# the3cloud/zktls

Measured on AMD Instinct MI355X. Metric: trace-cells/s, higher is better.
Workload: dtype u32

## Files before the change

### zktls_amd/csrc/hash.hip

```cpp
#include "poseidon2.cuh"
#include "poseidon2_coop.cuh"
#include "kernels.h"
#include "batch.h"
#include "p24chip.h"
#include "p24chip_rows.cuh"
#include "p2chip.h"

namespace zk {

hipError_t hash_upload_p2_tables(const P2Tables& t, hipStream_t s) { return p2_upload_tables(t, s); }

__device__ __forceinline__ uint32_t load_virtual(const LeafArgs& a, uint64_t row, uint32_t vc) {
    uint32_t off = vc;
#pragma unroll
    for (int m = 0; m < MAX_LEAF_MATS; m++) {
        if (m < a.nmats) {
            if (off < a.mats[m].width) return a.mats[m].ptr[row * a.mats[m].ld + off];
            off -= a.mats[m].width;
        }
    }
    return 0u;
}

__global__ void hash_rows16_kernel(LeafArgs a, uint32_t total_w);
struct hash_rows16_kernel_bargs { LeafArgs a; uint32_t total_w; static hash_rows16_kernel_bargs make(LeafArgs a, uint32_t total_w) { return hash_rows16_kernel_bargs{a, total_w}; } };
__global__ void hash_rows16_kernel_batch(const hash_rows16_kernel_bargs* __restrict__ zk_arr);
__global__ void compress_level16_kernel(const uint32_t* __restrict__ children, uint32_t* __restrict__ parents, uint32_t count);
struct compress_level16_kernel_bargs { const uint32_t* children; uint32_t* parents; uint32_t count; static compress_level16_kernel_bargs make(const uint32_t* children, uint32_t* parents, uint32_t count) { return compress_level16_kernel_bargs{children, parents, count}; } };
__global__ void compress_level16_kernel_batch(const compress_level16_kernel_bargs* __restrict__ zk_arr);
__global__ void compress_top16_kernel(uint32_t* tree, uint32_t count);
struct compress_top16_kernel_bargs { uint32_t* tree; uint32_t count; static compress_top16_kernel_bargs make(uint32_t* tree, uint32_t count) { return compress_top16_kernel_bargs{tree, count}; } };
__global__ void compress_top16_kernel_batch(const compress_top16_kernel_bargs* __restrict__ zk_arr);
__global__ void compress_sub16_kernel(uint32_t* tree, uint32_t count, uint32_t sub);
struct compress_sub16_kernel_bargs { uint32_t* tree; uint32_t count; uint32_t sub; static compress_sub16_kernel_bargs make(uint32_t* tree, uint32_t count, uint32_t sub) { return compress_sub16_kernel_bargs{tree, count, sub}; } };
__global__ void compress_sub16_kernel_batch(const compress_sub16_kernel_bargs* __restrict__ zk_arr);
__global__ void hash_sub16_kernel(LeafArgs a, uint32_t total_w, uint32_t sub);
struct hash_sub16_kernel_bargs { LeafArgs a; uint32_t total_w; uint32_t sub; static hash_sub16_kernel_bargs make(LeafArgs a, uint32_t total_w, uint32_t sub) { return hash_sub16_kernel_bargs{a, total_w, sub}; } };
__global__ void hash_sub16_kernel_batch(const hash_sub16_kernel_bargs* __restrict__ zk_arr);

__device__ __forceinline__ void hash_rows_generic_kernel_body(const LeafArgs& a, uint32_t total_w) {
    const uint64_t row = (uint64_t)blockIdx.x * blockDim.x + threadIdx.x;
    if (row >= a.height) return;
    uint32_t s[16];
#pragma unroll
    for (int i = 0; i < 16; i++) s[i] = 0u;
    for (uint32_t q = 0; q < total_w; q += 8) {
#pragma unroll
        for (int i = 0; i < 8; i++)
            if (q + i < total_w) s[i] = load_virtual(a, row, q + i);
        p2_permute_dev(s);
    }
    uint4* d = reinterpret_cast<uint4*>(a.digests + row * 8);
    d[0] = make_uint4(s[0], s[1], s[2], s[3]);
    d[1] = make_uint4(s[4], s[5], s[6], s[7]);
}
__global__ void __launch_bounds__(256) hash_rows_generic_kernel(LeafArgs a, uint32_t total_w) { hash_rows_generic_kernel_body(a, total_w); }
struct hash_rows_generic_kernel_bargs { LeafArgs a; uint32_t total_w; static hash_rows_generic_kernel_bargs make(LeafArgs a, uint32_t total_w) { return hash_rows_generic_kernel_bargs{a, total_w}; } };
__global__ void __launch_bounds__(256) hash_rows_generic_kernel_batch(const hash_rows_generic_kernel_bargs* __restrict__ zk_arr) { const hash_rows_generic_kernel_bargs& zk_b = zk_arr[blockIdx.z]; hash_rows_generic_kernel_body(zk_b.a, zk_b.total_w); }


template <bool MX>
__device__ __forceinline__ void hash_rows_vec_body(const uint32_t* __restrict__ mat, uint64_t ld, uint32_t width, uint64_t height, uint32_t* __restrict__ digests) {
    const uint64_t row = (uint64_t)blockIdx.x * blockDim.x + threadIdx.x;
    if (MX ? row - __lane_id() >= height : row >= height) return;
    const uint4* rp = reinterpret_cast<const uint4*>(mat + (row < height ? row : height - 1) * ld);
    uint32_t s[16];
#pragma unroll
    for (int i = 0; i < 16; i++) s[i] = 0u;
    for (uint32_t q = 0; q < width / 8; q++) {
        uint4 v0 = rp[2 * q], v1 = rp[2 * q + 1];
        s[0] = v0.x; s[1] = v0.y; s[2] = v0.z; s[3] = v0.w;
        s[4] = v1.x; s[5] = v1.y; s[6] = v1.z; s[7] = v1.w;
        if (MX) p2_permute_mx_dev(s); else p2_permute_dev(s);
    }
    if (width & 4u) {
        const uint4 v0 = rp[width / 4 - 1];
        s[0] = v0.x; s[1] = v0.y; s[2] = v0.z; s[3] = v0.w;
        if (MX) p2_permute_mx_dev(s); else p2_permute_dev(s);
    }
    if (row >= height) return;
    uint4* d = reinterpret_cast<uint4*>(digests + row * 8);
    d[0] = make_uint4(s[0], s[1], s[2], s[3]);
    d[1] = make_uint4(s[4], s[5], s[6], s[7]);
}
__device__ __forceinline__ void hash_rows_sponge_body(const uint32_t* __restrict__ mat, uint64_t ld, uint32_t width, uint64_t height, uint32_t* __restrict__ digests) {
    const uint64_t row = (uint64_t)blockIdx.x * blockDim.x + threadIdx.x;
    if (row - __lane_id() >= height) return;
    const uint4* rp = reinterpret_cast<const uint4*>(mat + (row < height ? row : height - 1) * ld);
    uint32_t s[16];
#pragma unroll
    for (int i = 0; i < 8; i++) { s[i] = 0u; s[8 + i] = (uint32_t)P2T.mx16.cap0[i]; }
    const uint32_t nb = width / 8, half = width & 4u;
    uint32_t q = 0;
    for (; q + 1 < nb; q++) {
        const uint4 v0 = rp[2 * q], v1 = rp[2 * q + 1];
        s[0] = v0.x; s[1] = v0.y; s[2] = v0.z; s[3] = v0.w;
        s[4] = v1.x; s[5] = v1.y; s[6] = v1.z; s[7] = v1.w;
        p2_permute_mx_form<P2MxForm::ABSORB>(s);
    }
    if (half && nb) {
        const uint4 v0 = rp[2 * q], v1 = rp[2 * q + 1];
        s[0] = v0.x; s[1] = v0.y; s[2] = v0.z; s[3] = v0.w;
        s[4] = v1.x; s[5] = v1.y; s[6] = v1.z; s[7] = v1.w;
        p2_permute_mx_form<P2MxForm::ABSORB_RATE>(s);
        q++;
    }
    if (width) {
        const uint4 v0 = rp[2 * q];
        s[0] = v0.x; s[1] = v0.y; s[2] = v0.z; s[3] = v0.w;
        if (!half) {
            const uint4 v1 = rp[2 * q + 1];
            s[4] = v1.x; s[5] = v1.y; s[6] = v1.z; s[7] = v1.w;
        }
        p2_permute_mx_form<P2MxForm::SQUEEZE>(s);
    }
    if (row >= height) return;
    uint4* d = reinterpret_cast<uint4*>(digests + row * 8);
    d[0] = make_uint4(s[0], s[1], s[2], s[3]);
    d[1] = make_uint4(s[4], s[5], s[6], s[7]);
}
__device__ __forceinline__ void hash_rows_vec_kernel_body(const uint32_t* __restrict__ mat, uint64_t ld, uint32_t width, uint64_t height, uint32_t* __restrict__ digests) { hash_rows_sponge_body(mat, ld, width, height, digests); }
__global__ void __launch_bounds__(256) __attribute__((amdgpu_waves_per_eu(5))) hash_rows_vec_kernel(const uint32_t* __restrict__ mat, uint64_t ld, uint32_t width, uint64_t height, uint32_t* __restrict__ digests) { hash_rows_vec_kernel_body(mat, ld, width, height, digests); }
struct hash_rows_vec_kernel_bargs { const uint32_t* mat; uint64_t ld; uint32_t width; uint64_t height; uint32_t* digests; static hash_rows_vec_kernel_bargs make(const uint32_t* mat, uint64_t ld, uint32_t width, uint64_t height, uint32_t* digests) { return hash_rows_vec_kernel_bargs{mat, ld, width, height, digests}; } };
__global__ void __launch_bounds__(256) __attribute__((amdgpu_waves_per_eu(5))) hash_rows_vec_kernel_batch(const hash_rows_vec_kernel_bargs* __restrict__ zk_arr) { const hash_rows_vec_kernel_bargs& zk_b = zk_arr[blockIdx.z]; hash_rows_vec_kernel_body(zk_b.mat, zk_b.ld, zk_b.width, zk_b.height, zk_b.digests); }
#ifdef ZKHIP_AB_HOOKS
__global__ void __launch_bounds__(256) hash_rows_vec_valu_kernel(const uint32_t* __restrict__ mat, uint64_t ld, uint32_t width, uint64_t height, uint32_t* __restrict__ digests) { hash_rows_vec_body<false>(mat, ld, width, height, digests); }
__global__ void __launch_bounds__(256) __attribute__((amdgpu_waves_per_eu(5))) hash_rows_vec_closed_kernel(const uint32_t* __restrict__ mat, uint64_t ld, uint32_t width, uint64_t height, uint32_t* __restrict__ digests) { hash_rows_vec_body<true>(mat, ld, width, height, digests); }
#endif

__device__ __forceinline__ void sponge_rows_vec(const LeafArgs& a, uint64_t row, uint32_t total_q, uint32_t s[16]) {
    int m = 0;
    uint32_t q = 0, nq = a.mats[0].width / 4;
    const uint4* rp = reinterpret_cast<const uint4*>(a.mats[0].ptr + row * a.mats[0].ld);
    for (uint32_t b = 0; b < total_q; b += 2) {
        while (q == nq) { m++; q = 0; nq = a.mats[m].width / 4; rp = reinterpret_cast<const uint4*>(a.mats[m].ptr + row * a.mats[m].ld); }
        const uint4 v0 = rp[q++];
        s[0] = v0.x; s[1] = v0.y; s[2] = v0.z; s[3] = v0.w;
        if (b + 1 < total_q) {
            while (q == nq) { m++; q = 0; nq = a.mats[m].width / 4; rp = reinterpret_cast<const uint4*>(a.mats[m].ptr + row * a.mats[m].ld); }
            const uint4 v1 = rp[q++];
            s[4] = v1.x; s[5] = v1.y; s[6] = v1.z; s[7] = v1.w;
        }
        p2_permute_dev(s);
    }
}
__device__ __forceinline__ void hash_rows_mvec_kernel_body(const LeafArgs& a, uint32_t total_q) {
    const uint64_t row = (uint64_t)blockIdx.x * blockDim.x + threadIdx.x;
    if (row >= a.height) return;
    uint32_t s[16];
#pragma unroll
    for (int i = 0; i < 16; i++) s[i] = 0u;
    sponge_rows_vec(a, row, total_q, s);
    uint4* d = reinterpret_cast<uint4*>(a.digests + row * 8);
    d[0] = make_uint4(s[0], s[1], s[2], s[3]);
    d[1] = make_uint4(s[4], s[5], s[6], s[7]);
}
__global__ void __launch_bounds__(256) hash_rows_mvec_kernel(LeafArgs a, uint32_t total_q) { hash_rows_mvec_kernel_body(a, total_q); }
struct hash_rows_mvec_kernel_bargs { LeafArgs a; uint32_t total_q; static hash_rows_mvec_kernel_bargs make(LeafArgs a, uint32_t total_q) { return hash_rows_mvec_kernel_bargs{a, total_q}; } };
__global__ void __launch_bounds__(256) hash_rows_mvec_kernel_batch(const hash_rows_mvec_kernel_bargs* __restrict__ zk_arr) { const hash_rows_mvec_kernel_bargs& zk_b = zk_arr[blockIdx.z]; hash_rows_mvec_kernel_body(zk_b.a, zk_b.total_q); }

__device__ __forceinline__ void compress_inject_mvec_kernel_body(const uint32_t* __restrict__ children, const LeafArgs& a, uint32_t total_q) {
    const uint64_t i = (uint64_t)blockIdx.x * blockDim.x + threadIdx.x;
    if (i >= a.height) return;
    const uint4* cp = reinterpret_cast<const uint4*>(children + 16 * i);
    const uint4 c0 = cp[0], c1 = cp[1], c2 = cp[2], c3 = cp[3];
    uint32_t s[16] = {c0.x, c0.y, c0.z, c0.w, c1.x, c1.y, c1.z, c1.w, c2.x, c2.y, c2.z, c2.w, c3.x, c3.y, c3.z, c3.w};
    uint32_t t[16];
#pragma unroll
    for (int k = 0; k < 16; k++) t[k] = 0u;
    p2_permute_dev(s);
    sponge_rows_vec(a, i, total_q, t);
#pragma unroll
    for (int k = 0; k < 8; k++) s[8 + k] = t[k];
    p2_permute_dev(s);
    uint4* d = reinterpret_cast<uint4*>(a.digests + i * 8);
    d[0] = make_uint4(s[0], s[1], s[2], s[3]);
    d[1] = make_uint4(s[4], s[5], s[6], s[7]);
}
__global__ void __launch_bounds__(256) compress_inject_mvec_kernel(const uint32_t* __restrict__ children, LeafArgs a, uint32_t total_q) { compress_inject_mvec_kernel_body(children, a, total_q); }
struct compress_inject_mvec_kernel_bargs { const uint32_t* children; LeafArgs a; uint32_t total_q; static compress_inject_mvec_kernel_bargs make(const uint32_t* children, LeafArgs a, uint32_t total_q) { return compress_inject_mvec_kernel_bargs{children, a, total_q}; } };
__global__ void __launch_bounds__(256) compress_inject_mvec_kernel_batch(const compress_inject_mvec_kernel_bargs* __restrict__ zk_arr) { const compress_inject_mvec_kernel_bargs& zk_b = zk_arr[blockIdx.z]; compress_inject_mvec_kernel_body(zk_b.children, zk_b.a, zk_b.total_q); }

static bool leaf_mats_vec(const LeafArgs& a) {
    for (int m = 0; m < a.nmats; m++) {
        const MatDesc& d = a.mats[m];
        if (d.width == 0 || d.width % 4 || d.ld % 4 || (reinterpret_cast<uintptr_t>(d.ptr) & 15)) return false;
    }
    return a.nmats >= 1;
}
hipError_t launch_compress_inject(const uint32_t* children, const LeafArgs& a, hipStream_t s) {
    if (a.height == 0) return hipSuccess;
    if (a.nmats < 1 || a.nmats > MAX_LEAF_MATS || !leaf_mats_vec(a)) return hipErrorInvalidValue;
    uint32_t total = 0;
    for (int m = 0; m < a.nmats; m++) total += a.mats[m].width;
    ZK_LAUNCH(compress_inject_mvec_kernel, compress_inject_mvec_kernel_batch, compress_inject_mvec_kernel_bargs, dim3((unsigned)((a.height + 255) / 256)), dim3(256), 0, s, children, a, total / 4);
    return hipGetLastError();
}
bool compress_inject_ok(const LeafArgs& a) { return a.height > coop_max_nodes() && leaf_mats_vec(a); }

hipError_t launch_hash_rows(const LeafArgs& a, hipStream_t s) {
    if (a.height == 0) return hipSuccess;
    if (a.nmats < 1 || a.nmats > MAX_LEAF_MATS) return hipErrorInvalidValue;
    uint32_t total = 0;
    for (int m = 0; m < a.nmats; m++) total += a.mats[m].width;
    if (a.height <= coop_max_nodes()) {
        const uint64_t threads = a.height * 16;
        ZK_LAUNCH(hash_rows16_kernel, hash_rows16_kernel_batch, hash_rows16_kernel_bargs, dim3((unsigned)((threads + 255) / 256)), dim3(256), 0, s, a, total);
        return hipGetLastError();
    }
    dim3 block(256), grid((unsigned)((a.height + 255) / 256));
    const MatDesc& m0 = a.mats[0];
    bool vec = a.nmats == 1 && m0.width % 4 == 0 && m0.ld % 4 == 0 &&
               (reinterpret_cast<uintptr_t>(m0.ptr) & 15) == 0;
#ifdef ZKHIP_AB_HOOKS
    static const bool valu = getenv("ZKHIP_HASH_VEC_VALU") != nullptr;
    if (vec && valu) {
        hash_rows_vec_valu_kernel<<<grid, block, 0, s>>>(m0.ptr, m0.ld, m0.width, a.height, a.digests);
        return hipGetLastError();
    }
    static const bool closed = getenv("ZKHIP_HASH_VEC_CLOSED") != nullptr;
    if (vec && closed) {
        hash_rows_vec_closed_kernel<<<grid, block, 0, s>>>(m0.ptr, m0.ld, m0.width, a.height, a.digests);
        return hipGetLastError();
    }
#endif
    if (vec)
        ZK_LAUNCH(hash_rows_vec_kernel, hash_rows_vec_kernel_batch, hash_rows_vec_kernel_bargs, grid, block, 0, s, m0.ptr, m0.ld, m0.width, a.height, a.digests);
    else if (leaf_mats_vec(a))
        ZK_LAUNCH(hash_rows_mvec_kernel, hash_rows_mvec_kernel_batch, hash_rows_mvec_kernel_bargs, grid, block, 0, s, a, total / 4);
    else
        ZK_LAUNCH(hash_rows_generic_kernel, hash_rows_generic_kernel_batch, hash_rows_generic_kernel_bargs, grid, block, 0, s, a, total);
    return hipGetLastError();
}

__device__ __forceinline__ void compress_node(const uint32_t* children, uint32_t* parent) {
    const uint4* cp = reinterpret_cast<const uint4*>(children);
    uint4 v0 = cp[0], v1 = cp[1], v2 = cp[2], v3 = cp[3];
    uint32_t s[16] = {v0.x, v0.y, v0.z, v0.w, v1.x, v1.y, v1.z, v1.w,
                      v2.x, v2.y, v2.z, v2.w, v3.x, v3.y, v3.z, v3.w};
    p2_permute_dev(s);
    uint4* d = reinterpret_cast<uint4*>(parent);
    d[0] = make_uint4(s[0], s[1], s[2], s[3]);
    d[1] = make_uint4(s[4], s[5], s[6], s[7]);
}

__device__ __forceinline__ void compress_level_kernel_body(const uint32_t* __restrict__ children, uint32_t* __restrict__ parents, uint64_t count) {
    const uint64_t i = (uint64_t)blockIdx.x * blockDim.x + threadIdx.x;
    if (i >= count) return;
    compress_node(children + 16 * i, parents + 8 * i);
}
__global__ void __launch_bounds__(256) compress_level_kernel(const uint32_t* __restrict__ children, uint32_t* __restrict__ parents, uint64_t count) { compress_level_kernel_body(children, parents, count); }
struct compress_level_kernel_bargs { const uint32_t* children; uint32_t* parents; uint64_t count; static compress_level_kernel_bargs make(const uint32_t* children, uint32_t* parents, uint64_t count) { return compress_level_kernel_bargs{children, parents, count}; } };
__global__ void __launch_bounds__(256) compress_level_kernel_batch(const compress_level_kernel_bargs* __restrict__ zk_arr) { const compress_level_kernel_bargs& zk_b = zk_arr[blockIdx.z]; compress_level_kernel_body(zk_b.children, zk_b.parents, zk_b.count); }

hipError_t launch_compress_level(const uint32_t* children, uint32_t* parents, uint64_t count, hipStream_t s) {
    if (count == 0) return hipSuccess;
    if (count <= coop_max_nodes()) {
        const uint64_t threads = count * 16;
        ZK_LAUNCH(compress_level16_kernel, compress_level16_kernel_batch, compress_level16_kernel_bargs, dim3((unsigned)((threads + 255) / 256)), dim3(256), 0, s, children, parents, (uint32_t)count);
        return hipGetLastError();
    }
    ZK_LAUNCH(compress_level_kernel, compress_level_kernel_batch, compress_level_kernel_bargs, dim3((unsigned)((count + 255) / 256)), dim3(256), 0, s, children, parents, count);
    return hipGetLastError();
}

__device__ __forceinline__ void inject_kernel_body(uint32_t* __restrict__ nodes, const uint32_t* __restrict__ extra, uint64_t count) {
    const uint64_t i = (uint64_t)blockIdx.x * blockDim.x + threadIdx.x;
    if (i >= count) return;
    const uint4* a = reinterpret_cast<const uint4*>(nodes + 8 * i);
    const uint4* b = reinterpret_cast<const uint4*>(extra + 8 * i);
    const uint4 v0 = a[0], v1 = a[1], v2 = b[0], v3 = b[1];
    uint32_t s[16] = {v0.x, v0.y, v0.z, v0.w, v1.x, v1.y, v1.z, v1.w, v2.x, v2.y, v2.z, v2.w, v3.x, v3.y, v3.z, v3.w};
    p2_permute_dev(s);
    uint4* d = reinterpret_cast<uint4*>(nodes + 8 * i);
    d[0] = make_uint4(s[0], s[1], s[2], s[3]);
    d[1] = make_uint4(s[4], s[5], s[6], s[7]);
}
__global__ void __launch_bounds__(256) inject_kernel(uint32_t* __restrict__ nodes, const uint32_t* __restrict__ extra, uint64_t count) { inject_kernel_body(nodes, extra, count); }
struct inject_kernel_bargs { uint32_t* nodes; const uint32_t* extra; uint64_t count; static inject_kernel_bargs make(uint32_t* nodes, const uint32_t* extra, uint64_t count) { return inject_kernel_bargs{nodes, extra, count}; } };
__global__ void __launch_bounds__(256) inject_kernel_batch(const inject_kernel_bargs* __restrict__ zk_arr) { const inject_kernel_bargs& zk_b = zk_arr[blockIdx.z]; inject_kernel_body(zk_b.nodes, zk_b.extra, zk_b.count); }

hipError_t launch_inject(uint32_t* nodes, const uint32_t* extra, uint64_t count, hipStream_t s) {
    if (count == 0) return hipSuccess;
    ZK_LAUNCH(inject_kernel, inject_kernel_batch, inject_kernel_bargs, dim3((unsigned)((count + 255) / 256)), dim3(256), 0, s, nodes, extra, count);
    return hipGetLastError();
}

__device__ __forceinline__ void compress_top_kernel_body(uint32_t* tree, uint32_t count) {
    uint32_t* level = tree;
    for (uint32_t n = count; n > 1; n >>= 1) {
        uint32_t* next = level + 8 * (size_t)n;
        for (uint32_t i = threadIdx.x; i < n / 2; i += blockDim.x) compress_node(level + 16 * (size_t)i, next + 8 * (size_t)i);
        __threadfence_block();
        __syncthreads();
        level = next;
    }
}
__global__ void __launch_bounds__(1024) compress_top_kernel(uint32_t* tree, uint32_t count) { compress_top_kernel_body(tree, count); }
struct compress_top_kernel_bargs { uint32_t* tree; uint32_t count; static compress_top_kernel_bargs make(uint32_t* tree, uint32_t count) { return compress_top_kernel_bargs{tree, count}; } };
__global__ void __launch_bounds__(1024) compress_top_kernel_batch(const compress_top_kernel_bargs* __restrict__ zk_arr) { const compress_top_kernel_bargs& zk_b = zk_arr[blockIdx.z]; compress_top_kernel_body(zk_b.tree, zk_b.count); }

hipError_t launch_compress_top(uint32_t* tree, uint32_t count, hipStream_t s) {
    if (count <= 1) return hipSuccess;
    if (count > COOP_TOP_NODES) return hipErrorInvalidValue;
    unsigned threads = count * 8 < 64 ? 64 : (count * 8 > 1024 ? 1024 : count * 8);
    ZK_LAUNCH(compress_top16_kernel, compress_top16_kernel_batch, compress_top16_kernel_bargs, dim3(1), dim3(threads), 0, s, tree, count);
    return hipGetLastError();
}

hipError_t launch_hash_sub(const LeafArgs& a, uint32_t sub, hipStream_t s) {
    if (sub < 2 || (sub & (sub - 1)) || a.height % sub || a.height > COOP_MAX_NODES || a.nmats < 1 || a.nmats > MAX_LEAF_MATS) return hipErrorInvalidValue;
    uint32_t total = 0;
    for (int m = 0; m < a.nmats; m++) total += a.mats[m].width;
    unsigned threads = sub * 8 < 64 ? 64 : (sub * 8 > 1024 ? 1024 : sub * 8);
    ZK_LAUNCH(hash_sub16_kernel, hash_sub16_kernel_batch, hash_sub16_kernel_bargs, dim3((unsigned)(a.height / sub)), dim3(threads), 0, s, a, total, sub);
    return hipGetLastError();
}
hipError_t launch_compress_sub(uint32_t* tree, uint32_t count, uint32_t sub, hipStream_t s) {
    if (sub < 2 || (sub & (sub - 1)) || count % sub || count > COOP_MAX_NODES) return hipErrorInvalidValue;
    unsigned threads = sub * 8 < 64 ? 64 : (sub * 8 > 1024 ? 1024 : sub * 8);
    ZK_LAUNCH(compress_sub16_kernel, compress_sub16_kernel_batch, compress_sub16_kernel_bargs, dim3(count / sub), dim3(threads), 0, s, tree, count, sub);
    return hipGetLastError();
}

__device__ __forceinline__ void compress_level16_kernel_body(const uint32_t* __restrict__ children, uint32_t* __restrict__ parents, uint32_t count) {
    const uint32_t gid = blockIdx.x * blockDim.x + threadIdx.x;
    const uint32_t node = gid >> 4;
    const int lane16 = threadIdx.x & 15;
    if (node >= count) return;
    const CoopConsts k = coop_load_consts(lane16);
    const uint32_t x = coop_permute(children[16 * (size_t)node + lane16], lane16, k);
    if (lane16 < 8) parents[8 * (size_t)node + lane16] = x;
}
__global__ void __launch_bounds__(256) compress_level16_kernel(const uint32_t* __restrict__ children, uint32_t* __restrict__ parents, uint32_t count) { compress_level16_kernel_body(children, parents, count); }
__global__ void __launch_bounds__(256) compress_level16_kernel_batch(const compress_level16_kernel_bargs* __restrict__ zk_arr) { const compress_level16_kernel_bargs& zk_b = zk_arr[blockIdx.z]; compress_level16_kernel_body(zk_b.children, zk_b.parents, zk_b.count); }

__device__ __forceinline__ void compress_top16_kernel_body(uint32_t* tree, uint32_t count) {
    const int lane16 = threadIdx.x & 15;
    const uint32_t grp = threadIdx.x >> 4, ngrp = blockDim.x >> 4;
    const CoopConsts k = coop_load_consts(lane16);
    uint32_t* level = tree;
    for (uint32_t n = count; n > 1; n >>= 1) {
        uint32_t* next = level + 8 * (size_t)n;
        for (uint32_t i = grp; i < n / 2; i += ngrp) {
            const uint32_t x = coop_permute(level[16 * (size_t)i + lane16], lane16, k);
            if (lane16 < 8) next[8 * (size_t)i + lane16] = x;
        }
        __threadfence_block();
        __syncthreads();
        level = next;
    }
}
__global__ void __launch_bounds__(1024) compress_top16_kernel(uint32_t* tree, uint32_t count) { compress_top16_kernel_body(tree, count); }
__global__ void __launch_bounds__(1024) compress_top16_kernel_batch(const compress_top16_kernel_bargs* __restrict__ zk_arr) { const compress_top16_kernel_bargs& zk_b = zk_arr[blockIdx.z]; compress_top16_kernel_body(zk_b.tree, zk_b.count); }

__device__ __forceinline__ void compress_sub16_kernel_body(uint32_t* tree, uint32_t count, uint32_t sub) {
    const int lane16 = threadIdx.x & 15;
    const uint32_t grp = threadIdx.x >> 4, ngrp = blockDim.x >> 4;
    const CoopConsts k = coop_load_consts(lane16);
    uint32_t* level = tree;
    uint32_t n = count, mine = sub;
    while (mine > 1) {
        uint32_t* next = level + 8 * (size_t)n;
        const size_t in0 = (size_t)blockIdx.x * mine, out0 = (size_t)blockIdx.x * (mine / 2);
        for (uint32_t i = grp; i < mine / 2; i += ngrp) {
            const uint32_t x = coop_permute(level[16 * (in0 / 2 + i) + lane16], lane16, k);
            if (lane16 < 8) next[8 * (out0 + i) + lane16] = x;
        }
        __threadfence_block();
        __syncthreads();
        level = next; n >>= 1; mine >>= 1;
    }
}
__global__ void __launch_bounds__(1024) compress_sub16_kernel(uint32_t* tree, uint32_t count, uint32_t sub) { compress_sub16_kernel_body(tree, count, sub); }
__global__ void __launch_bounds__(1024) compress_sub16_kernel_batch(const compress_sub16_kernel_bargs* __restrict__ zk_arr) { const compress_sub16_kernel_bargs& zk_b = zk_arr[blockIdx.z]; compress_sub16_kernel_body(zk_b.tree, zk_b.count, zk_b.sub); }
// ... 887 lines not shown
```

### zktls_amd/csrc/poseidon2.cuh

```cuda
#pragma once
#include "babybear.cuh"
#include "p2_params.h"

namespace zk {

struct P2Consts {
    uint32_t ext_rc[8][16];
    uint32_t int_rc[13];
    uint32_t diag[16];
    uint32_t ext_rcm[8][16];
    uint32_t int_rcm[13];
};
struct P2Raw {
    uint32_t ext16[8][16], int16[13], diag16[16];
    uint32_t ext24[8][24], int24[21], diag24[24];
};
constexpr P2Consts make_p2_consts(const P2Raw& raw) {
    P2Consts k{};
    for (int r = 0; r < 8; r++)
        for (int i = 0; i < 16; i++) k.ext_rc[r][i] = to_monty(raw.ext16[r][i]);
    for (int r = 0; r < 13; r++) k.int_rc[r] = to_monty(raw.int16[r]);
    for (int i = 0; i < 16; i++) k.diag[i] = to_monty(raw.diag16[i]);
    for (int r = 0; r < 8; r++)
        for (int i = 0; i < 16; i++) k.ext_rcm[r][i] = k.ext_rc[r][i] - P;
// ... 442 lines not shown
}
ZK_D void p2_m4_hl_dev(uint32_t& x0, uint32_t& x1, uint32_t& x2, uint32_t& x3) {
    const uint32_t t0 = dadd(x0, x1);
    const uint32_t t1 = dadd(x2, x3);
    const uint32_t t2 = dadd(ddbl(x1), t1);
    const uint32_t t3 = dadd(ddbl(x3), t0);
    const uint32_t t4 = dadd(ddbl(ddbl(t1)), t3);
    const uint32_t t5 = dadd(ddbl(ddbl(t0)), t2);
    x0 = dadd(t3, t5);
    x1 = t5;
    x2 = dadd(t2, t4);
    x3 = t4;
}
ZK_D void p2_external_linear_dev(uint32_t s[16]) {
    p2_m4_dev(s[0], s[1], s[2], s[3]);
    p2_m4_dev(s[4], s[5], s[6], s[7]);
    p2_m4_dev(s[8], s[9], s[10], s[11]);
    p2_m4_dev(s[12], s[13], s[14], s[15]);
    const uint32_t t0 = dadd(dadd(s[0], s[4]), dadd(s[8], s[12]));
    const uint32_t t1 = dadd(dadd(s[1], s[5]), dadd(s[9], s[13]));
    const uint32_t t2 = dadd(dadd(s[2], s[6]), dadd(s[10], s[14]));
    const uint32_t t3 = dadd(dadd(s[3], s[7]), dadd(s[11], s[15]));
#pragma unroll
    for (int b = 0; b < 16; b += 4) {
        s[b] = dadd(s[b], t0);
        s[b + 1] = dadd(s[b + 1], t1);
        s[b + 2] = dadd(s[b + 2], t2);
        s[b + 3] = dadd(s[b + 3], t3);
    }
}
#ifndef P2_INT_UNROLL
#define P2_INT_UNROLL 1
#endif
ZK_D int32_t p2_sbox_signed(int32_t t) {
    const int32_t x2 = dsmont(t, t);
    const int32_t x4 = dsmont(x2, x2);
    const int32_t x6 = dsmont(x4, x2);
    return dsmont(x6, t);
}
ZK_D void p2_internal_round_dev(int32_t v[16], int r, int32_t sh) {
    v[0] = p2_sbox_signed(v[0]);
    int64_t T = 0;
#pragma unroll
    for (int j = 0; j < 16; j++) T = dsmac_uniform(v[j], sh, T);
    const int32_t sum = dsmred(T);
    int64_t T2 = dsmac_s(sum, P2IK.k_sum, 0);
    v[0] = dsmred(dsmac_s(v[0], P2IK.diag[0], T2 + (int64_t)P2IK.rc_fold[r]));
#pragma unroll
    for (int i = 1; i < 16; i++) v[i] = dsmred(dsmac_s(v[i], P2IK.diag[i], T2));
}
ZK_D void p2_internal_pair_dev(int32_t v[16], int r, int32_t sh24) {
    int64_t A = 0;
#pragma unroll
    for (int i = 1; i < 16; i++) A = dsmac_uniform(v[i], P2PK.rs_mul[i], A);
    const int32_t u = p2_sbox_signed(v[0]);
    int64_t T = 0;
    T = dsmac_uniform(u, sh24, T);
#pragma unroll
    for (int j = 1; j < 16; j++) T = dsmac_uniform(v[j], sh24, T);
    const int32_t sum_t = dsmred(T);
    const int32_t v0 = dsmred(dsmac_s(u, P2IK.diag[0], dsmac_s(sum_t, P2PK.k_sum_a, 0) + (int64_t)P2IK.rc_fold[r]));
    A = dsmac_s(sum_t, P2PK.c15, A);
    const int32_t u2 = p2_sbox_signed(v0);
    A = dsmac_uniform(u2, P2PK.rs_mul[0], A);
    const int64_t T2 = dsmac_s(dsmred(A), P2PK.k_sum_b, 0);
    v[0] = dsmred(dsmac_s(u2, P2IK.diag[0], T2 + (int64_t)P2IK.rc_fold[r + 1]));
#pragma unroll
    for (int i = 1; i < 16; i++) v[i] = dsmred(dsmac_s(v[i], P2PK.d2[i], dsmac_s(sum_t, P2PK.e[i], T2)));
}
ZK_D void p2_internal_rounds_dev(uint32_t s[16]) {
    int32_t v[16];
#pragma unroll
    for (int i = 0; i < 16; i++) v[i] = (int32_t)s[i];
    int32_t sh, sh24;
    asm volatile("s_mov_b32 %0, 0x8000000" : "=s"(sh));
    asm volatile("s_mov_b32 %0, 0x1000000" : "=s"(sh24));
    p2_internal_round_dev(v, 0, sh);
    if (P2PK.pair) {
#pragma unroll P2_INT_UNROLL
        for (int r = 1; r < 13; r += 2) p2_internal_pair_dev(v, r, sh24);
    } else {
#pragma unroll P2_INT_UNROLL
        for (int r = 1; r < 13; r++) p2_internal_round_dev(v, r, sh);
    }
#pragma unroll
    for (int i = 0; i < 16; i++) s[i] = dcanon(v[i]);
}
ZK_D uint32_t p2_sbox_fold_dev(int32_t t, int64_t fold_biased) {
    const int32_t x2 = dsmont(t, t);
    const int32_t x4 = dsmont(x2, x2);
    const int32_t x6 = dsmont(x4, x2);
    return dred(dmred_lazy((uint64_t)dsmac(x6, t, fold_biased)));
}
ZK_D void p2_external_linear_signed_dev(uint32_t s[16]) {
    p2_m4_dev(s[0], s[1], s[2], s[3]);
    p2_m4_dev(s[4], s[5], s[6], s[7]);
    p2_m4_dev(s[8], s[9], s[10], s[11]);
    p2_m4_dev(s[12], s[13], s[14], s[15]);
    const uint32_t t0 = dadd(dadd(s[0], s[4]), dadd(s[8], s[12])) - P;
    const uint32_t t1 = dadd(dadd(s[1], s[5]), dadd(s[9], s[13])) - P;
    const uint32_t t2 = dadd(dadd(s[2], s[6]), dadd(s[10], s[14])) - P;
    const uint32_t t3 = dadd(dadd(s[3], s[7]), dadd(s[11], s[15])) - P;
#pragma unroll
    for (int b = 0; b < 16; b += 4) {
        s[b] += t0;
        s[b + 1] += t1;
        s[b + 2] += t2;
        s[b + 3] += t3;
    }
}
ZK_D void p2_permute_dev(uint32_t s[16]) {
    p2_external_linear_dev(s);
#pragma unroll
    for (int i = 0; i < 16; i++) s[i] += P2K.ext_rcm[0][i];
#pragma unroll 1
    for (int r = 0; r < 4; r++) {
#pragma unroll
        for (int i = 0; i < 16; i++) s[i] = p2_sbox_fold_dev((int32_t)s[i], P2EF.c[r][i]);
        p2_external_linear_signed_dev(s);
    }
    p2_internal_rounds_dev(s);
#pragma unroll
    for (int i = 0; i < 16; i++) s[i] += P2K.ext_rcm[4][i];
#pragma unroll 1
    for (int r = 4; r < 8; r++) {
#pragma unroll
        for (int i = 0; i < 16; i++) s[i] = p2_sbox_fold_dev((int32_t)s[i], P2EF.c[r][i]);
        p2_external_linear_signed_dev(s);
    }
#pragma unroll
    for (int i = 0; i < 16; i++) s[i] = dcanon((int32_t)s[i]);
}

typedef int p2mx_v4i __attribute__((ext_vector_type(4)));
typedef int p2mx_v16i __attribute__((ext_vector_type(16)));
constexpr int32_t MX_C24 = centered((uint32_t)(((uint64_t)1 << 56) % P));
constexpr uint32_t p2_me_entry(int i, int j) {
    return ((i >> 2) == (j >> 2) ? 2u : 1u) * (uint32_t)(0x1132u >> (4 * ((j - i) & 3)) & 15u);
}
constexpr uint32_t p2_mx_a_word(int lane, int idx) {
    const int m = lane & 31, h = lane >> 5, mb = idx >> 3, kb = (idx >> 2) & 1, r = idx & 3;
    return p2_me_entry(mx_elem((m >> 2) & 1, 4 * mb + (m >> 3)), mx_elem(h, 4 * kb + r)) << (8 * (m & 3));
}
struct P2MxA { uint32_t w[64][16]; };
constexpr P2MxA make_p2_mx_a() {
    P2MxA a{};
    for (int l = 0; l < 64; l++)
        for (int i = 0; i < 16; i++) a.w[l][i] = p2_mx_a_word(l, i);
    return a;
}
static_assert(p2_me_entry(0, 0) == 4 && p2_me_entry(0, 1) == 6 && p2_me_entry(1, 0) == 2 && p2_me_entry(3, 0) == 6 && p2_me_entry(4, 1) == 3,
              "M_E entries");
static __constant__ P2MxA d_p2_mx_a = make_p2_mx_a();
ZK_D void p2_mx_load_a(p2mx_v4i a[4]) {
    const uint4* p = reinterpret_cast<const uint4*>(d_p2_mx_a.w[__lane_id()]);
#pragma unroll
    for (int i = 0; i < 4; i++) { const uint4 v = p[i]; a[i] = p2mx_v4i{(int)v.x, (int)v.y, (int)v.z, (int)v.w}; }
}
ZK_D void p2_mx_layer_block(const uint32_t d[8], const p2mx_v4i a[4], int32_t w[8], int mb) {
    const p2mx_v4i b0 = {(int)d[0], (int)d[1], (int)d[2], (int)d[3]}, b1 = {(int)d[4], (int)d[5], (int)d[6], (int)d[7]};
    p2mx_v16i y = {};
    y = __builtin_amdgcn_mfma_i32_32x32x32_i8(a[2 * mb], b0, y, 0, 0, 0);
    y = __builtin_amdgcn_mfma_i32_32x32x32_i8(a[2 * mb + 1], b1, y, 0, 0, 0);
#pragma unroll
    for (int e = 0; e < 4; e++) {
        const uint32_t L = (uint32_t)y[4 * e] + ((uint32_t)y[4 * e + 1] << 8) + ((uint32_t)y[4 * e + 2] << 16);
        w[4 * mb + e] = dsmred((int64_t)((uint64_t)L << 32) + (int64_t)y[4 * e + 3] * MX_C24);
    }
}
ZK_D void p2_mx_layer(const uint32_t d[8], const p2mx_v4i a[4], int32_t w[8]) {
    p2_mx_layer_block(d, a, w, 0);
    p2_mx_layer_block(d, a, w, 1);
}
ZK_D uint32_t p2_sbox_mx_dev(int32_t t, int64_t fold_mx) {
    const int32_t x2 = dsmont(t, t);
    const int32_t x4 = dsmont(x2, x2);
    const int32_t x6 = dsmont(x4, x2);
    return dmred_lazy((uint64_t)dsmac(x6, t, fold_mx)) ^ 0x80808080u;
}
ZK_D void p2_mx_swap(uint32_t x[8], uint32_t y[8]) {
#pragma unroll
    for (int q = 0; q < 8; q++) {
        const auto r = __builtin_amdgcn_permlane32_swap(x[q], y[q], false, false);
        x[q] = r[0]; y[q] = r[1];
    }
}
ZK_D void p2_mx_full_rounds(int32_t wa[8], int32_t wb[8], int r0, int h) {
    p2mx_v4i a[4];
    p2_mx_load_a(a);
#pragma unroll 1
    for (int r = r0; r < r0 + 4; r++) {
        const int64_t* f = P2T.mx16.fold[r][h];
        uint32_t d[8];
#pragma unroll
        for (int q = 0; q < 8; q++) d[q] = p2_sbox_mx_dev(wa[q], f[q]);
        p2_mx_layer(d, a, wa);
#pragma unroll
        for (int q = 0; q < 8; q++) d[q] = p2_sbox_mx_dev(wb[q], f[q]);
        p2_mx_layer(d, a, wb);
    }
}
template <int BLOCKS>
ZK_D void p2_mx_last_rounds(int32_t wa[8], int32_t wb[8], int h, const int64_t* f7) {
    p2mx_v4i a[4];
    p2_mx_load_a(a);
    uint32_t d[8];
#pragma unroll 1
    for (int r = 4; r < 7; r++) {
        const int64_t* f = P2T.mx16.fold[r][h];
#pragma unroll
        for (int q = 0; q < 8; q++) d[q] = p2_sbox_mx_dev(wa[q], f[q]);
        p2_mx_layer(d, a, wa);
#pragma unroll
        for (int q = 0; q < 8; q++) d[q] = p2_sbox_mx_dev(wb[q], f[q]);
        p2_mx_layer(d, a, wb);
    }
#pragma unroll
    for (int q = 0; q < 8; q++) d[q] = p2_sbox_mx_dev(wa[q], f7[q]);
    if (BLOCKS & 1) p2_mx_layer_block(d, a, wa, 0);
    if (BLOCKS & 2) p2_mx_layer_block(d, a, wa, 1);
#pragma unroll
    for (int q = 0; q < 8; q++) d[q] = p2_sbox_mx_dev(wb[q], f7[q]);
    if (BLOCKS & 1) p2_mx_layer_block(d, a, wb, 0);
    if (BLOCKS & 2) p2_mx_layer_block(d, a, wb, 1);
}
enum class P2MxForm { CLOSED, ABSORB, ABSORB_RATE, SQUEEZE };
template <P2MxForm F>
ZK_D void p2_permute_mx_form(uint32_t s[16]) {
    constexpr bool SPONGE = F != P2MxForm::CLOSED;
    const int h = __lane_id() >> 5;
    uint32_t x[8], y[8];
    int32_t wa[8], wb[8];
#pragma unroll
    for (int q = 0; q < 8; q++) { x[q] = s[mx_elem(0, q)]; y[q] = s[mx_elem(1, q)]; }
    p2_mx_swap(x, y);
    {
        const uint32_t* c = P2T.mx16.in0[h];
        uint32_t da[8], db[8];
        p2mx_v4i a[4];
        p2_mx_load_a(a);
#pragma unroll
        for (int q = 0; q < 8; q++) {
            const uint32_t cq = SPONGE && q >= 4 ? 0x80808080u : c[q];
            da[q] = (x[q] + cq) ^ 0x80808080u; db[q] = (y[q] + cq) ^ 0x80808080u;
        }
        p2_mx_layer(da, a, wa);
        p2_mx_layer(db, a, wb);
    }
    p2_mx_full_rounds(wa, wb, 0, h);
#pragma unroll
    for (int q = 0; q < 8; q++) { x[q] = (uint32_t)wa[q]; y[q] = (uint32_t)wb[q]; }
    p2_mx_swap(x, y);
#pragma unroll
    for (int q = 0; q < 8; q++) { s[mx_elem(0, q)] = x[q]; s[mx_elem(1, q)] = y[q]; }
    p2_internal_rounds_dev(s);
#pragma unroll
    for (int q = 0; q < 8; q++) { x[q] = s[mx_elem(0, q)] + P2K.ext_rcm[4][mx_elem(0, q)]; y[q] = s[mx_elem(1, q)] + P2K.ext_rcm[4][mx_elem(1, q)]; }
    p2_mx_swap(x, y);
#pragma unroll
    for (int q = 0; q < 8; q++) { wa[q] = (int32_t)x[q]; wb[q] = (int32_t)y[q]; }
    if (!SPONGE) {
        p2_mx_full_rounds(wa, wb, 4, h);
#pragma unroll
        for (int q = 0; q < 8; q++) { x[q] = dcanon(wa[q]); y[q] = dcanon(wb[q]); }
        p2_mx_swap(x, y);
#pragma unroll
        for (int q = 0; q < 8; q++) { s[mx_elem(0, q)] = x[q]; s[mx_elem(1, q)] = y[q]; }
    } else {
        constexpr int BLOCKS = F == P2MxForm::SQUEEZE ? 1 : F == P2MxForm::ABSORB ? 2 : 3;
        p2_mx_last_rounds<BLOCKS>(wa, wb, h, F == P2MxForm::SQUEEZE ? P2T.mx16.fold[7][h] : P2T.mx16.fold7a[h]);
#pragma unroll
        for (int q = 0; q < 8; q++) {
            if (!(BLOCKS >> (q >> 2) & 1)) continue;
            const uint32_t xa = q < 4 ? dcanon(wa[q]) : (uint32_t)wa[q], yb = q < 4 ? dcanon(wb[q]) : (uint32_t)wb[q];
            const auto r = __builtin_amdgcn_permlane32_swap(xa, yb, false, false);
            s[mx_elem(0, q)] = r[0]; s[mx_elem(1, q)] = r[1];
        }
        if (F == P2MxForm::ABSORB) {
#pragma unroll
            for (int i = 0; i < 8; i++) s[i] = 0u;
        }
    }
}
ZK_D void p2_permute_mx_dev(uint32_t s[16]) { p2_permute_mx_form<P2MxForm::CLOSED>(s); }
#endif

#if defined(__HIPCC__)
ZK_D void p24_external_linear_dev(uint32_t s[24]) {
#pragma unroll
    for (int b = 0; b < 24; b += 4) p2_m4_hl_dev(s[b], s[b + 1], s[b + 2], s[b + 3]);
    uint32_t t[4];
#pragma unroll
    for (int k = 0; k < 4; k++)
        t[k] = dadd(dadd(dadd(s[k], s[4 + k]), dadd(s[8 + k], s[12 + k])), dadd(s[16 + k], s[20 + k]));
#pragma unroll
    for (int i = 0; i < 24; i++) s[i] = dadd(s[i], t[i & 3]);
}
ZK_D void p24_internal_rounds_dev(uint32_t s[24]) {
    int32_t v[24];
#pragma unroll
    for (int i = 0; i < 24; i++) v[i] = (int32_t)s[i];
    int32_t sh;
    asm volatile("s_mov_b32 %0, 0x4000000" : "=s"(sh));
#pragma unroll P2_INT_UNROLL
    for (int r = 0; r < 21; r++) {
        v[0] = p2_sbox_signed(v[0]);
        int64_t T = 0;
#pragma unroll
        for (int j = 0; j < 24; j++) T = dsmac_uniform(v[j], sh, T);
        const int32_t sum = dsmred(T);
        int64_t T2 = dsmac_s(sum, P24IK.k_sum, 0);
        v[0] = dsmred(dsmac_s(v[0], P24IK.diag[0], T2 + (int64_t)P24IK.rc_fold[r]));
#pragma unroll
        for (int i = 1; i < 24; i++) v[i] = dsmred(dsmac_s(v[i], P24IK.diag[i], T2));
    }
#pragma unroll
    for (int i = 0; i < 24; i++) s[i] = dcanon(v[i]);
}
ZK_D void p24_external_linear_signed_dev(uint32_t s[24]) {
#pragma unroll
    for (int b = 0; b < 24; b += 4) p2_m4_hl_dev(s[b], s[b + 1], s[b + 2], s[b + 3]);
    uint32_t t[4];
#pragma unroll
    for (int k = 0; k < 4; k++)
        t[k] = dadd(dadd(dadd(s[k], s[4 + k]), dadd(s[8 + k], s[12 + k])), dadd(s[16 + k], s[20 + k])) - P;
#pragma unroll
    for (int i = 0; i < 24; i++) s[i] += t[i & 3];
}
ZK_D void p24_permute_dev(uint32_t s[24]) {
    p24_external_linear_dev(s);
#pragma unroll
    for (int i = 0; i < 24; i++) s[i] += P24K.ext_rcm[0][i];
#pragma unroll 1
    for (int r = 0; r < 4; r++) {
#pragma unroll
        for (int i = 0; i < 24; i++) s[i] = p2_sbox_fold_dev((int32_t)s[i], P24EF.c[r][i]);
        p24_external_linear_signed_dev(s);
    }
    p24_internal_rounds_dev(s);
#pragma unroll
    for (int i = 0; i < 24; i++) s[i] += P24K.ext_rcm[4][i];
#pragma unroll 1
    for (int r = 4; r < 8; r++) {
#pragma unroll
        for (int i = 0; i < 24; i++) s[i] = p2_sbox_fold_dev((int32_t)s[i], P24EF.c[r][i]);
        p24_external_linear_signed_dev(s);
    }
#pragma unroll
    for (int i = 0; i < 24; i++) s[i] = dcanon((int32_t)s[i]);
}
#endif

inline void p24_external_linear(uint32_t s[24]) {
    for (int b = 0; b < 24; b += 4) p2_m4_hl(s[b], s[b + 1], s[b + 2], s[b + 3]);
    uint32_t t[4];
    for (int k = 0; k < 4; k++) {
        t[k] = 0;
        for (int b = 0; b < 24; b += 4) t[k] = fadd(t[k], s[b + k]);
    }
    for (int i = 0; i < 24; i++) s[i] = fadd(s[i], t[i & 3]);
}
inline void p24_permute(uint32_t s[24]) {
    p24_external_linear(s);
    for (int r = 0; r < 4; r++) {
        for (int i = 0; i < 24; i++) s[i] = p2_sbox(fadd(s[i], P24HK.ext_rc[r][i]));
        p24_external_linear(s);
    }
    for (int r = 0; r < 21; r++) {
        s[0] = p2_sbox(fadd(s[0], P24HK.int_rc[r]));
        uint32_t sum = 0;
        for (int i = 0; i < 24; i++) sum = fadd(sum, s[i]);
        for (int i = 0; i < 24; i++) s[i] = fadd(fmul(s[i], P24HK.diag[i]), sum);
    }
    for (int r = 4; r < 8; r++) {
        for (int i = 0; i < 24; i++) s[i] = p2_sbox(fadd(s[i], P24HK.ext_rc[r][i]));
        p24_external_linear(s);
    }
}

ZK_HD constexpr void p2_compress(const uint32_t l[8], const uint32_t r[8], uint32_t out[8]) {
    uint32_t s[16] = {};
    for (int i = 0; i < 8; i++) { s[i] = l[i]; s[8 + i] = r[i]; }
    p2_permute(s);
    for (int i = 0; i < 8; i++) out[i] = s[i];
}

}
```

Measured before the change: 21.37 billion.

## Derive MFMA A operand in registers and stage Poseidon2 constants in LDS

The sponge row-hash kernel now builds the MFMA A operand (M_E ⊗ I_4 layout) from a closed-form expression per lane instead of loading it from constant memory, with a static_assert checking it against the table. It also copies the mx16 round-constant tables into shared memory once per block and reads fold/in0 constants from LDS. Both aim to cut scalar/constant-memory load traffic and latency inside the permutation rounds. The cost is a block-wide sync plus LDS usage that may lower occupancy, and some extra ALU work to rebuild the A operand. The old path stays reachable behind an environment-variable hook.

```diff
diff --git a/zktls_amd/csrc/hash.hip b/zktls_amd/csrc/hash.hip
--- a/zktls_amd/csrc/hash.hip
+++ b/zktls_amd/csrc/hash.hip
@@ -83,7 +83,12 @@
     d[0] = make_uint4(s[0], s[1], s[2], s[3]);
     d[1] = make_uint4(s[4], s[5], s[6], s[7]);
 }
+template <bool LEAN>
 __device__ __forceinline__ void hash_rows_sponge_body(const uint32_t* __restrict__ mat, uint64_t ld, uint32_t width, uint64_t height, uint32_t* __restrict__ digests) {
+    constexpr int OPT = LEAN ? P2MX_A_DERIVED | P2MX_LDS : 0;
+    __shared__ P2MxConsts lk_store;
+    const P2MxConsts* lk = nullptr;
+    if (LEAN) { p2_mx_stage_consts(&lk_store); lk = &lk_store; }
     const uint64_t row = (uint64_t)blockIdx.x * blockDim.x + threadIdx.x;
     if (row - __lane_id() >= height) return;
     const uint4* rp = reinterpret_cast<const uint4*>(mat + (row < height ? row : height - 1) * ld);
@@ -96,13 +101,13 @@
         const uint4 v0 = rp[2 * q], v1 = rp[2 * q + 1];
         s[0] = v0.x; s[1] = v0.y; s[2] = v0.z; s[3] = v0.w;
         s[4] = v1.x; s[5] = v1.y; s[6] = v1.z; s[7] = v1.w;
-        p2_permute_mx_form<P2MxForm::ABSORB>(s);
+        p2_permute_mx_form<P2MxForm::ABSORB, OPT>(s, lk);
     }
     if (half && nb) {
         const uint4 v0 = rp[2 * q], v1 = rp[2 * q + 1];
         s[0] = v0.x; s[1] = v0.y; s[2] = v0.z; s[3] = v0.w;
         s[4] = v1.x; s[5] = v1.y; s[6] = v1.z; s[7] = v1.w;
-        p2_permute_mx_form<P2MxForm::ABSORB_RATE>(s);
+        p2_permute_mx_form<P2MxForm::ABSORB_RATE, OPT>(s, lk);
         q++;
     }
     if (width) {
@@ -112,20 +117,21 @@
             const uint4 v1 = rp[2 * q + 1];
             s[4] = v1.x; s[5] = v1.y; s[6] = v1.z; s[7] = v1.w;
         }
-        p2_permute_mx_form<P2MxForm::SQUEEZE>(s);
+        p2_permute_mx_form<P2MxForm::SQUEEZE, OPT>(s, lk);
     }
     if (row >= height) return;
     uint4* d = reinterpret_cast<uint4*>(digests + row * 8);
     d[0] = make_uint4(s[0], s[1], s[2], s[3]);
     d[1] = make_uint4(s[4], s[5], s[6], s[7]);
 }
-__device__ __forceinline__ void hash_rows_vec_kernel_body(const uint32_t* __restrict__ mat, uint64_t ld, uint32_t width, uint64_t height, uint32_t* __restrict__ digests) { hash_rows_sponge_body(mat, ld, width, height, digests); }
+__device__ __forceinline__ void hash_rows_vec_kernel_body(const uint32_t* __restrict__ mat, uint64_t ld, uint32_t width, uint64_t height, uint32_t* __restrict__ digests) { hash_rows_sponge_body<true>(mat, ld, width, height, digests); }
 __global__ void __launch_bounds__(256) __attribute__((amdgpu_waves_per_eu(5))) hash_rows_vec_kernel(const uint32_t* __restrict__ mat, uint64_t ld, uint32_t width, uint64_t height, uint32_t* __restrict__ digests) { hash_rows_vec_kernel_body(mat, ld, width, height, digests); }
 struct hash_rows_vec_kernel_bargs { const uint32_t* mat; uint64_t ld; uint32_t width; uint64_t height; uint32_t* digests; static hash_rows_vec_kernel_bargs make(const uint32_t* mat, uint64_t ld, uint32_t width, uint64_t height, uint32_t* digests) { return hash_rows_vec_kernel_bargs{mat, ld, width, height, digests}; } };
 __global__ void __launch_bounds__(256) __attribute__((amdgpu_waves_per_eu(5))) hash_rows_vec_kernel_batch(const hash_rows_vec_kernel_bargs* __restrict__ zk_arr) { const hash_rows_vec_kernel_bargs& zk_b = zk_arr[blockIdx.z]; hash_rows_vec_kernel_body(zk_b.mat, zk_b.ld, zk_b.width, zk_b.height, zk_b.digests); }
 #ifdef ZKHIP_AB_HOOKS
 __global__ void __launch_bounds__(256) hash_rows_vec_valu_kernel(const uint32_t* __restrict__ mat, uint64_t ld, uint32_t width, uint64_t height, uint32_t* __restrict__ digests) { hash_rows_vec_body<false>(mat, ld, width, height, digests); }
 __global__ void __launch_bounds__(256) __attribute__((amdgpu_waves_per_eu(5))) hash_rows_vec_closed_kernel(const uint32_t* __restrict__ mat, uint64_t ld, uint32_t width, uint64_t height, uint32_t* __restrict__ digests) { hash_rows_vec_body<true>(mat, ld, width, height, digests); }
+__global__ void __launch_bounds__(256) __attribute__((amdgpu_waves_per_eu(5))) hash_rows_vec_parent_kernel(const uint32_t* __restrict__ mat, uint64_t ld, uint32_t width, uint64_t height, uint32_t* __restrict__ digests) { hash_rows_sponge_body<false>(mat, ld, width, height, digests); }
 #endif
 
 __device__ __forceinline__ void sponge_rows_vec(const LeafArgs& a, uint64_t row, uint32_t total_q, uint32_t s[16]) {
@@ -221,6 +227,11 @@
     static const bool closed = getenv("ZKHIP_HASH_VEC_CLOSED") != nullptr;
     if (vec && closed) {
         hash_rows_vec_closed_kernel<<<grid, block, 0, s>>>(m0.ptr, m0.ld, m0.width, a.height, a.digests);
+        return hipGetLastError();
+    }
+    static const bool parent = getenv("ZKHIP_HASH_VEC_PARENT") != nullptr;
+    if (vec && parent) {
+        hash_rows_vec_parent_kernel<<<grid, block, 0, s>>>(m0.ptr, m0.ld, m0.width, a.height, a.digests);
         return hipGetLastError();
     }
 #endif
diff --git a/zktls_amd/csrc/poseidon2.cuh b/zktls_amd/csrc/poseidon2.cuh
--- a/zktls_amd/csrc/poseidon2.cuh
+++ b/zktls_amd/csrc/poseidon2.cuh
@@ -618,10 +618,40 @@
 static_assert(p2_me_entry(0, 0) == 4 && p2_me_entry(0, 1) == 6 && p2_me_entry(1, 0) == 2 && p2_me_entry(3, 0) == 6 && p2_me_entry(4, 1) == 3,
               "M_E entries");
 static __constant__ P2MxA d_p2_mx_a = make_p2_mx_a();
+constexpr uint32_t p2_mx_a_base(int lane, int r) { return (0x1132u >> (4 * ((r - ((lane & 31) >> 3)) & 3)) & 15u) << (8 * (lane & 3)); }
+constexpr uint32_t p2_mx_a_shift(int lane) { return ((lane >> 2) & 1) == (lane >> 5) ? 1u : 0u; }
+constexpr bool p2_mx_a_derived_ok() {
+    for (int l = 0; l < 64; l++)
+        for (int i = 0; i < 16; i++)
+            if (p2_mx_a_word(l, i) != p2_mx_a_base(l, i & 3) << ((i >> 3) == ((i >> 2) & 1) ? p2_mx_a_shift(l) : 0u)) return false;
+    return true;
+}
+static_assert(p2_mx_a_derived_ok(), "the A operand's derived form differs from M_E (x) I_4 in the MFMA layout");
+enum : int { P2MX_A_DERIVED = 1, P2MX_LDS = 2 };
+template <int OPT>
 ZK_D void p2_mx_load_a(p2mx_v4i a[4]) {
-    const uint4* p = reinterpret_cast<const uint4*>(d_p2_mx_a.w[__lane_id()]);
-#pragma unroll
-    for (int i = 0; i < 4; i++) { const uint4 v = p[i]; a[i] = p2mx_v4i{(int)v.x, (int)v.y, (int)v.z, (int)v.w}; }
+    if constexpr (OPT & P2MX_A_DERIVED) {
+        const int l = (int)__lane_id();
+        const uint32_t s = p2_mx_a_shift(l);
+        p2mx_v4i b1, b2;
+#pragma unroll
+        for (int r = 0; r < 4; r++) { const uint32_t b = p2_mx_a_base(l, r); b1[r] = (int)b; b2[r] = (int)(b << s); }
+        a[0] = b2; a[1] = b1; a[2] = b1; a[3] = b2;
+    } else {
+        const uint4* p = reinterpret_cast<const uint4*>(d_p2_mx_a.w[__lane_id()]);
+#pragma unroll
+        for (int i = 0; i < 4; i++) { const uint4 v = p[i]; a[i] = p2mx_v4i{(int)v.x, (int)v.y, (int)v.z, (int)v.w}; }
+    }
+}
+ZK_D void p2_mx_stage_consts(P2MxConsts* lk) {
+    static_assert(sizeof(P2MxConsts) % 16 == 0, "P2MxConsts is copied in 16-byte words");
+    const uint4* src = reinterpret_cast<const uint4*>(&P2T.mx16);
+    for (unsigned i = threadIdx.x; i < sizeof(P2MxConsts) / 16; i += blockDim.x) reinterpret_cast<uint4*>(lk)[i] = src[i];
+    __syncthreads();
+}
+template <int OPT>
+ZK_D const P2MxConsts& p2_mx_consts(const P2MxConsts* lk) {
+    if constexpr (OPT & P2MX_LDS) return *lk; else return P2T.mx16;
 }
 ZK_D void p2_mx_layer_block(const uint32_t d[8], const p2mx_v4i a[4], int32_t w[8], int mb) {
     const p2mx_v4i b0 = {(int)d[0], (int)d[1], (int)d[2], (int)d[3]}, b1 = {(int)d[4], (int)d[5], (int)d[6], (int)d[7]};
@@ -651,12 +681,13 @@
         x[q] = r[0]; y[q] = r[1];
     }
 }
-ZK_D void p2_mx_full_rounds(int32_t wa[8], int32_t wb[8], int r0, int h) {
+template <int OPT>
+ZK_D void p2_mx_full_rounds(int32_t wa[8], int32_t wb[8], int r0, int h, const P2MxConsts& k) {
     p2mx_v4i a[4];
-    p2_mx_load_a(a);
+    p2_mx_load_a<OPT>(a);
 #pragma unroll 1
     for (int r = r0; r < r0 + 4; r++) {
-        const int64_t* f = P2T.mx16.fold[r][h];
+        const int64_t* f = k.fold[r][h];
         uint32_t d[8];
 #pragma unroll
         for (int q = 0; q < 8; q++) d[q] = p2_sbox_mx_dev(wa[q], f[q]);
@@ -666,14 +697,14 @@
         p2_mx_layer(d, a, wb);
     }
 }
-template <int BLOCKS>
-ZK_D void p2_mx_last_rounds(int32_t wa[8], int32_t wb[8], int h, const int64_t* f7) {
+template <int BLOCKS, int OPT>
+ZK_D void p2_mx_last_rounds(int32_t wa[8], int32_t wb[8], int h, const P2MxConsts& k, const int64_t* f7) {
     p2mx_v4i a[4];
-    p2_mx_load_a(a);
+    p2_mx_load_a<OPT>(a);
     uint32_t d[8];
 #pragma unroll 1
     for (int r = 4; r < 7; r++) {
-        const int64_t* f = P2T.mx16.fold[r][h];
+        const int64_t* f = k.fold[r][h];
 #pragma unroll
         for (int q = 0; q < 8; q++) d[q] = p2_sbox_mx_dev(wa[q], f[q]);
         p2_mx_layer(d, a, wa);
@@ -691,20 +722,21 @@
     if (BLOCKS & 2) p2_mx_layer_block(d, a, wb, 1);
 }
 enum class P2MxForm { CLOSED, ABSORB, ABSORB_RATE, SQUEEZE };
-template <P2MxForm F>
-ZK_D void p2_permute_mx_form(uint32_t s[16]) {
+template <P2MxForm F, int OPT = 0>
+ZK_D void p2_permute_mx_form(uint32_t s[16], const P2MxConsts* lk = nullptr) {
     constexpr bool SPONGE = F != P2MxForm::CLOSED;
     const int h = __lane_id() >> 5;
+    const P2MxConsts& k = p2_mx_consts<OPT>(lk);
     uint32_t x[8], y[8];
     int32_t wa[8], wb[8];
 #pragma unroll
     for (int q = 0; q < 8; q++) { x[q] = s[mx_elem(0, q)]; y[q] = s[mx_elem(1, q)]; }
     p2_mx_swap(x, y);
     {
-        const uint32_t* c = P2T.mx16.in0[h];
+        const uint32_t* c = k.in0[h];
         uint32_t da[8], db[8];
         p2mx_v4i a[4];
-        p2_mx_load_a(a);
+        p2_mx_load_a<OPT>(a);
 #pragma unroll
         for (int q = 0; q < 8; q++) {
             const uint32_t cq = SPONGE && q >= 4 ? 0x80808080u : c[q];
@@ -713,7 +745,7 @@
         p2_mx_layer(da, a, wa);
         p2_mx_layer(db, a, wb);
     }
-    p2_mx_full_rounds(wa, wb, 0, h);
+    p2_mx_full_rounds<OPT>(wa, wb, 0, h, k);
 #pragma unroll
     for (int q = 0; q < 8; q++) { x[q] = (uint32_t)wa[q]; y[q] = (uint32_t)wb[q]; }
     p2_mx_swap(x, y);
@@ -726,7 +758,7 @@
 #pragma unroll
     for (int q = 0; q < 8; q++) { wa[q] = (int32_t)x[q]; wb[q] = (int32_t)y[q]; }
     if (!SPONGE) {
-        p2_mx_full_rounds(wa, wb, 4, h);
+        p2_mx_full_rounds<OPT>(wa, wb, 4, h, k);
 #pragma unroll
         for (int q = 0; q < 8; q++) { x[q] = dcanon(wa[q]); y[q] = dcanon(wb[q]); }
         p2_mx_swap(x, y);
@@ -734,7 +766,7 @@
         for (int q = 0; q < 8; q++) { s[mx_elem(0, q)] = x[q]; s[mx_elem(1, q)] = y[q]; }
     } else {
         constexpr int BLOCKS = F == P2MxForm::SQUEEZE ? 1 : F == P2MxForm::ABSORB ? 2 : 3;
-        p2_mx_last_rounds<BLOCKS>(wa, wb, h, F == P2MxForm::SQUEEZE ? P2T.mx16.fold[7][h] : P2T.mx16.fold7a[h]);
+        p2_mx_last_rounds<BLOCKS, OPT>(wa, wb, h, k, F == P2MxForm::SQUEEZE ? k.fold[7][h] : k.fold7a[h]);
 #pragma unroll
         for (int q = 0; q < 8; q++) {
             if (!(BLOCKS >> (q >> 2) & 1)) continue;
```

New measurement: 21.70 billion, median of 6. +1.5%, better.
